# aconverse/ffmpeg-heaac

Measured on AMD Instinct MI355X. Metric: HE-AAC frames/s (batched), higher is better.
Workload: dtype f32; 1 GPU; HE-AACv2 stereo 48 kHz, 256 k-frame batch; frames_per_gpu=262144, pcm=f32, bytes_per_frame=85284, parallelism=frames sharded by index, no collective

## Files before the change

### ffmpeg-heaac_amd/csrc/k_he.hip

```cpp
#include <stdlib.h>
#include <type_traits>
#include "k_core.h"
#include "k_core2.h"
#include "kernels.h"

#include "k_hf.h"

#define ANA_WAVES 8
#define ANA_POOL  3456

struct AnaLds {
    CoreLds core;
    float qmf_ds[320];
    float rot[64];
    float pool[ANA_WAVES][ANA_POOL];
};

__device__ __forceinline__ void qmf_analysis_wave(const float *qmf_ds, const float *rot,
                                                  const float *c16, const float *c32,
                                                  const float *x, float *u, float *g_W, int lane)
{
    {
        const int k = lane;
        const float w0 = qmf_ds[k], w1 = qmf_ds[k + 64], w2 = qmf_ds[k + 128],
                    w3 = qmf_ds[k + 192], w4 = qmf_ds[k + 256];
        for (int i = 0; i < 32; i++) {
            const float *xs = x + 32 * i + 319 - k;
            const float f = w0 * xs[0] + w1 * xs[-64] + w2 * xs[-128] + w3 * xs[-192] + w4 * xs[-256];
            u[i * 65 + k] = f;
        }
    }
    wave_sync();
    if (lane < 32) {
        const float *f = u + lane * 65;
        float o[64];
        imdct128_reg([&](int j) -> float {
                         if (j == 0)  return f[0];
                         if (j == 63) return f[32];
                         return (j & 1) ? f[(j + 1) >> 1] : -f[64 - (j >> 1)];
                     }, o, rot, c16, c32);
        float *row = u + lane * 65;
#pragma unroll
        for (int k = 0; k < 32; k++) {
            row[2 * k]     = -o[63 - k];
            row[2 * k + 1] = o[k];
        }
    }
    wave_sync();
    for (int t = lane; t < 2048; t += WAVE)
        g_W[t] = u[(t >> 6) * 65 + (t & 63)];
    wave_sync();
}

#define CA_WAVES 7
#define CA_U     2080

struct CaWave {
    float tu[2 * 2 * C2_TSTRIDE];
    float x1[1312];
    float x0u1[CA_U];
};
static_assert(CA_U >= 1312, "x of channel 0 fits under u of channel 1");
static_assert(CA_U <= 2 * 2 * C2_TSTRIDE, "u rows of channel 0 lie over the core's transpose regions");

template <bool STRIDED, class... Hold>
__global__ __launch_bounds__(CA_WAVES * WAVE)
void k_core_ana(const float *__restrict__ g_tab, const uint16_t *__restrict__ g_rev,
                const float *__restrict__ g_coeffs, const HeaacIcs *__restrict__ g_ics,
                const float *g_state_in, float *g_state_out, int state_words,
                int ncore, int off_saved0, int off_sbr0,
                float *__restrict__ g_W, float scale, unsigned long long n_units, unsigned long long rstride, Hold... hold)
{
    constexpr bool HOLD = sizeof...(Hold) != 0;
    static_assert(STRIDED || !HOLD, "the batch form has no hold mask");
    auto rec = [&](unsigned long long u) -> unsigned long long {
        if constexpr (STRIDED) return (u / ncore) * rstride * ncore + u % ncore;
        else return u;
    };
    __shared__ float s_cos[TB_ROT2048];
    __shared__ float s_rot256[128];
    __shared__ float s_wshort[256];
    __shared__ uint16_t s_kA512[512], s_kA64[64];
    __shared__ float s_qmf_ds[320];
    __shared__ float s_rot[64];
    __shared__ CaWave S[CA_WAVES];
    static_assert(TB_SINE_SHORT == TB_KBD_SHORT + 128, "the two short windows are copied as one run");
    for (int i = threadIdx.x; i < TB_ROT2048; i += blockDim.x) s_cos[i] = g_tab[i];
    for (int i = threadIdx.x; i < 128; i += blockDim.x) s_rot256[i] = g_tab[TB_ROT256 + i];
    for (int i = threadIdx.x; i < 256; i += blockDim.x) s_wshort[i] = g_tab[TB_KBD_SHORT + i];
    for (int k = threadIdx.x; k < 512; k += blockDim.x) {
        const int e = g_rev[RV_512 + k];
        s_kA512[(e & 15) * 32 + (e >> 4)] = (uint16_t)k;
    }
    for (int k = threadIdx.x; k < 64; k += blockDim.x) {
        const int e = g_rev[RV_64 + k];
        s_kA64[(e & 15) * 4 + (e >> 4)] = (uint16_t)k;
    }
    for (int i = threadIdx.x; i < 320; i += blockDim.x) s_qmf_ds[i] = g_tab[TB_QMF_DS + i];
    for (int i = threadIdx.x; i < 64; i += blockDim.x)  s_rot[i] = g_tab[TB_ROT128A + i];
    __syncthreads();
    const CoreTabs L = { s_cos, g_tab + TB_ROT2048, s_rot256, g_tab + TB_KBD_LONG, g_tab + TB_SINE_LONG,
                         s_wshort, s_wshort + 128,
                         reinterpret_cast<const float2 *>(g_tab + TB_ROTA512), reinterpret_cast<const float2 *>(g_tab + TB_ROTA64),
                         s_kA512, s_kA64 };
    const int wave = __builtin_amdgcn_readfirstlane(threadIdx.x / WAVE), lane0 = threadIdx.x % WAVE;
    CaWave &w = S[wave];
    cpx *T0 = reinterpret_cast<cpx *>(w.tu), *T1 = T0 + C2_TSTRIDE;
    const float *c16 = s_cos + TB_COS16, *c32 = s_cos + TB_COS32;
    const unsigned long long pairs = (n_units + 1) / 2;
    LongTw tw;
    core2_load_long_twiddles(L, lane0 & 31, tw);
    for (unsigned long long pr = (unsigned long long)blockIdx.x * CA_WAVES + wave; pr < pairs;
         pr += (unsigned long long)gridDim.x * CA_WAVES) {
        const unsigned long long u0 = 2 * pr;
        const bool have1 = u0 + 1 < n_units;
        const unsigned long long u1 = have1 ? u0 + 1 : u0;
        unsigned long long r0 = rec(u0), r1 = rec(u1);
        [[maybe_unused]] bool run0 = true, run1 = have1;
        if constexpr (HOLD) {
            const uint8_t *g_hold = hold_mask(hold...);
            run0 = __builtin_amdgcn_readfirstlane((int)g_hold[(u0 / ncore) * rstride]) == 0;
            run1 = have1 && __builtin_amdgcn_readfirstlane((int)g_hold[(u1 / ncore) * rstride]) == 0;
            if (!run0 && !run1) continue;
            if (!run0) r0 = r1;
            if (!run1) r1 = r0;
        }
        const HeaacIcs ics0 = g_ics[r0], ics1 = g_ics[r1];
        int lane = opaque(lane0);
        core2_stage_coeffs(reinterpret_cast<float *>(T0), g_coeffs + r0 * 1024, lane);
        core2_stage_coeffs(reinterpret_cast<float *>(T1), g_coeffs + r1 * 1024, lane);
        wave_sync();
        {
            const int half = lane >> 5, hl = lane & 31;
            const bool eight = (half ? ics1.window_sequence[0] : ics0.window_sequence[0]) == HEAAC_EIGHT_SHORT_SEQUENCE;
            cpx *T = half ? T1 : T0;
            imdct_half_regs_tw<true>(L, reinterpret_cast<const float *>(T), T, eight, hl, tw);
        }
#pragma unroll
        for (int c = 0; c < 2; c++) {
            if (c == 1 && !have1) break;
            if constexpr (HOLD) {
                if (!(c ? run1 : run0)) continue;
            }
            const unsigned long long u = c ? u1 : u0;
            const unsigned long long f = u / ncore;
            const int ch = (int)(u - f * ncore);
            const float *st_in = g_state_in + f * state_words;
            float *st_out = g_state_out + f * state_words;
            const int off_saved = off_saved0 + ch * HEAAC_ST_SAVED;
            const int off_sbr = off_sbr0 + ch * HEAAC_ST_SBR;
            float *x = c ? w.x1 : w.x0u1;
            const float *xh_in = st_in + off_sbr + HEAAC_SBR_XHIST;
            float xh[5];
#pragma unroll
            for (int t = 0; t < 5; t++) xh[t] = 64 * t + lane < 288 ? xh_in[64 * t + lane] : 0.0f;
            const float *buf = reinterpret_cast<const float *>(c ? T1 : T0);
            const OverlapHbm ov{ st_in + off_saved, st_out + off_saved };
            if (scale != 1.0f)
                core2_window(L, c ? ics1 : ics0, 0.0f, buf, ov, lane, [&](int q, float v) { x[288 + q] = v * scale; });
            else
                core2_window(L, c ? ics1 : ics0, 0.0f, buf, ov, lane, [&](int q, float v) { x[288 + q] = v; });
#pragma unroll
            for (int t = 0; t < 5; t++) if (64 * t + lane < 288) x[64 * t + lane] = xh[t];
        }
        wave_sync();
        lane = opaque(lane);
#pragma unroll
        for (int c = 0; c < 2; c++) {
            if (c == 1 && !have1) break;
            if constexpr (HOLD) {
                if (!(c ? run1 : run0)) continue;
            }
            const unsigned long long u = c ? u1 : u0;
            const unsigned long long f = u / ncore;
            const int ch = (int)(u - f * ncore);
            float *xh_out = g_state_out + f * state_words + off_sbr0 + ch * HEAAC_ST_SBR + HEAAC_SBR_XHIST;
            const float *x = c ? w.x1 : w.x0u1;
            float *uu = c ? w.x0u1 : w.tu;
#pragma unroll
            for (int t = 0; t < 5; t++) if (64 * t + lane < 288) xh_out[64 * t + lane] = x[1024 + 64 * t + lane];
            const int k = lane;
            const float w0 = s_qmf_ds[k], w1 = s_qmf_ds[k + 64], w2 = s_qmf_ds[k + 128],
                        w3 = s_qmf_ds[k + 192], w4 = s_qmf_ds[k + 256];
            const float *xk = x + 319 - k;
            v2f a1 = v2f{xk[-64], xk[-32]}, a2 = v2f{xk[-128], xk[-96]}, a3 = v2f{xk[-192], xk[-160]},
                a4 = v2f{xk[-256], xk[-224]};
#pragma unroll
            for (int i = 0; i < 32; i += 2) {
                const v2f a0 = v2f{xk[32 * i], xk[32 * i + 32]};
                const v2f f = bc(w0) * a0 + bc(w1) * a1 + bc(w2) * a2 + bc(w3) * a3 + bc(w4) * a4;
                uu[i * 65 + k] = f.x;
                uu[(i + 1) * 65 + k] = f.y;
                a4 = a3; a3 = a2; a2 = a1; a1 = a0;
            }
        }
        wave_sync();
        lane = opaque(lane);
        {
            float *row = (lane >> 5 ? w.x0u1 : w.tu) + (lane & 31) * 65;
            const float *f = row;
            float o[64];
            imdct128_reg([&](int j) -> float {
                             if (j == 0)  return f[0];
                             if (j == 63) return f[32];
                             return (j & 1) ? f[(j + 1) >> 1] : -f[64 - (j >> 1)];
                         }, o, s_rot, c16, c32);
#pragma unroll
            for (int k = 0; k < 32; k++) {
                row[2 * k]     = -o[63 - k];
                row[2 * k + 1] = o[k];
            }
        }
        wave_sync();
#pragma unroll
        for (int c = 0; c < 2; c++) {
            if (c == 1 && !have1) break;
            if constexpr (HOLD) {
                if (!(c ? run1 : run0)) continue;
            }
            const float *uu = c ? w.x0u1 : w.tu;
            float *Wo = g_W + (c ? u1 : u0) * 2048;
#pragma unroll
            for (int it = 0; it < 8; it++) {
                const int r = 4 * it + (lane >> 4), q = 4 * (lane & 15);
                const float *sr = uu + r * 65 + q;
                *reinterpret_cast<float4 *>(Wo + r * 64 + q) = make_float4(sr[0], sr[1], sr[2], sr[3]);
            }
        }
        wave_sync();
    }
}

template <bool STRIDED, class... Hold>
__global__ __launch_bounds__(HF_WAVES * WAVE)
void k_hfadj(const float *__restrict__ g_tab,
             const HeaacSbrFrame *__restrict__ g_sbr, const HeaacSbrHeader *__restrict__ g_hdr, unsigned n_hdr,
             const float *g_W, const float *g_state_in, float *g_state_out, int state_words,
             int ncore, int off_sbr0, float *g_X, unsigned long long n_units, unsigned *g_queue,
             unsigned char *__restrict__ g_xtop, unsigned long long rstride, Hold... hold)
{
    static_assert(STRIDED || sizeof...(Hold) == 0, "the batch form has no hold mask");
    __shared__ float s_xlow[HF_WAVES][HF_XLOW_WORDS], s_aux[HF_WAVES][HF_AUX_WORDS], s_rec[HF_WAVES][HF_REC_WORDS];
    __shared__ float s_noise[1024];
    wg_copy_f4(s_noise, g_tab + TB_NOISE, 1024);
    __syncthreads();
    const int wave = __builtin_amdgcn_readfirstlane(threadIdx.x / WAVE), lane = threadIdx.x % WAVE;
    const HfWave S = hf_wave_view(s_xlow[wave], s_aux[wave], s_rec[wave]);
    FrameFeed<1> feed;
    feed.init((unsigned long long)blockIdx.x * HF_WAVES + wave, (unsigned long long)gridDim.x * HF_WAVES, g_queue, lane);
    while (feed.cur * 2 < n_units) {
        const unsigned long long ub = feed.cur * 2;
        feed.request(lane);
      for (int qi = 0; qi < 2 && ub + qi < n_units; qi++) {
        const unsigned long long u = ub + qi;
        const unsigned long long f = u / ncore;
        if constexpr (sizeof...(Hold) != 0) {
            if (__builtin_amdgcn_readfirstlane((int)hold_mask(hold...)[f * rstride])) continue;
        }
        const int ch = (int)(u - f * ncore);
        const int off = off_sbr0 + ch * HEAAC_ST_SBR;
        const HeaacSbrFrame *sbr = STRIDED ? &g_sbr[f * rstride] : &g_sbr[f];
        v2f *Xc = reinterpret_cast<v2f *>(g_X + (f * 2 + ch) * HE_X_CHANNEL);
        int xb = 64;
        hf_channel(S, s_noise, sbr, g_hdr, n_hdr, ch, g_W + u * 2048,
                   g_state_in + f * state_words + off, g_state_out + f * state_words + off, lane,
                   [&](int i, float re, float im) {
                       if (i == 0 && g_xtop) {
                           const int top16 = (S.h.kx + S.h.m + 15) & ~15;
                           const int t_old = S.c[ch].t_env_num_env_old;
                           const bool zero = 2 * t_old - 32 <= 0 || (int)sbr->kx_old + (int)sbr->m_old <= top16;
                           xb = __builtin_amdgcn_readfirstlane(zero && top16 < 64 ? top16 : 64);
                           if (lane == 0 && xb != 64) g_xtop[f * 2 + ch] = (unsigned char)xb;
                       }
                       if (lane < xb) __builtin_nontemporal_store(v2f{re, im}, Xc + i * 64 + lane);
                   });
      }
        feed.advance();
    }
}

#define SYN_WAVES 6
#define VB_STRIDE 129
#define VB_ROWS   41

#define SYN_WAVES_F32 7
struct SynWave {
    __attribute__((aligned(16))) float vb[VB_ROWS * VB_STRIDE + 3];
};
template <int NW>
struct SynLdsT {
    float win[640];
    float rot[64];
    float c16[8], c32[12];
    SynWave w[NW];
};
typedef SynLdsT<SYN_WAVES> SynLds;

#ifdef HEAAC_STAMPS
#define SSTAMP(i) TL_STAMP(i, (i) == 0)
#else
#define SSTAMP(i) do {} while (0)
#endif

__device__ __forceinline__ float lane_xor1(float v)
{
    return __int_as_float(__builtin_amdgcn_update_dpp(0, __float_as_int(v), 0xB1, 0xF, 0xF, false));
}

struct SynIn {
// ... 499 lines not shown
#pragma nounroll
                        for (int q = lane; q < 1024; q += WAVE) o[q * nout] = 0;
                    }
                    continue;
                }
                move = fresh;
                fresh = true;
            }
            if (move) {
                float h[9];
#pragma unroll
                for (int k = 0; k < 9; k++) h[k] = vb[k * DS_STRIDE + lane];
#pragma unroll
                for (int k = 0; k < 9; k++) vb[(32 + k) * DS_STRIDE + lane] = h[k];
            }
            const unsigned long long u = (unsigned long long)t * n_streams + st, r = st * T + t;
            const float *X0 = g_X + (u * 2 + ch) * HE_X_CHANNEL;
            if constexpr (FMT == HEAAC_PCM_F32_PLANAR) {
                float *o = reinterpret_cast<float *>(g_pcm) + (r * nout + ch) * 1024;
                synth_ds_channel<false, false>(S, vb, X0, nullptr, nullptr, nullptr, scale, bias, lane,
                                               [&](int i, int nn, float v) { o[32 * i + nn] = v; });
            } else {
                int16_t *o = reinterpret_cast<int16_t *>(g_pcm) + r * 1024 * nout + ch;
                synth_ds_channel<false, false>(S, vb, X0, nullptr, nullptr, nullptr, scale, bias, lane,
                                               [&](int i, int nn, float v) { o[(32 * i + nn) * nout] = (int16_t)pcm_int16<FMT>(v); });
            }
        }
        if constexpr (HOLD) {
            const int row0 = fresh ? 0 : 32;
            for (int q = lane; q < 576; q += WAVE) v_out[q] = vb[(row0 + (q >> 6)) * DS_STRIDE + (q & 63)];
        } else {
            for (int q = lane; q < 576; q += WAVE) v_out[q] = vb[(q >> 6) * DS_STRIDE + (q & 63)];
        }
        wave_sync();
    }
}

static int he_grid(unsigned long long units, int per_block)
{
    unsigned long long g = (units + per_block - 1) / per_block;
    if (g > 256) g = 256;
    if (g < 1) g = 1;
    return (int)g;
}

static bool he_fused()
{
#ifdef HEAAC_TUNING
    static const bool fused = []() { const char *e = getenv("HEAAC_HE_UNFUSED"); return !(e && e[0] == '1'); }();
    return fused;
#else
    return true;
#endif
}

extern "C" int heaac_launch_he(const float *d_tab, const uint16_t *d_rev, int cfg,
                               const float *d_coeffs, const HeaacIcs *d_ics,
                               const HeaacSbrFrame *d_sbr, const HeaacSbrHeader *d_hdr, unsigned n_hdr,
                               const HeaacPsFrame *d_ps,
                               const float *d_state_in, float *d_state_out,
                               void *d_pcm, int pcm_format,
                               float *d_ws_W, float *d_ws_X, unsigned *d_queue,
                               unsigned char *d_xtop, const float *d_zero,
                               size_t n, size_t pcm_frame0, int flags, hipStream_t s)
{
    const int ncore = cfg == HEAAC_CFG_HEV1 ? 2 : 1;
    const int nout  = cfg == HEAAC_CFG_HEV1_MONO ? 1 : 2;
    int words, off_saved0 = 0, off_sbr0, off_syn0;
    if (cfg == HEAAC_CFG_HEV1) {
        words = HEAAC_STATE_WORDS_HEV1; off_sbr0 = 2 * HEAAC_ST_SAVED; off_syn0 = off_sbr0 + 2 * HEAAC_ST_SBR;
    } else if (cfg == HEAAC_CFG_HEV1_MONO) {
        words = HEAAC_STATE_WORDS_HEV1_MONO; off_sbr0 = HEAAC_ST_SAVED; off_syn0 = off_sbr0 + HEAAC_ST_SBR;
    } else if (cfg == HEAAC_CFG_HEV2) {
        words = HEAAC_STATE_WORDS_HEV2; off_sbr0 = HEAAC_ST_SAVED; off_syn0 = off_sbr0 + HEAAC_ST_SBR;
    } else
        return HEAAC_ERR_ARG;
    const unsigned long long units = (unsigned long long)n * ncore;
    const bool simd = pcm_format == HEAAC_PCM_S16_INTERLEAVED_SSE2;
    const float sf_scale = simd ? -1.0f / 1024.0f : HEAAC_SF_SCALE;

    if (hipMemsetAsync(d_queue, 0, 64, s) != hipSuccess) return HEAAC_ERR_HIP;
    if (hipMemsetAsync(d_xtop, 64, 2 * n, s) != hipSuccess) return HEAAC_ERR_HIP;
    hipLaunchKernelGGL(k_core_ana<false>, dim3(he_grid((units + 1) / 2, CA_WAVES)), dim3(CA_WAVES * WAVE), 0, s,
                       d_tab, d_rev, d_coeffs, d_ics, d_state_in, d_state_out, words, ncore,
                       off_saved0, off_sbr0, d_ws_W, 1 / (-1024 * sf_scale), units, 1ull);
    if (cfg == HEAAC_CFG_HEV2 && he_fused()) {
        const int off_ps = off_syn0 + 2 * HEAAC_ST_SYNTH;
        int rc = heaac_launch_hfps(d_tab, d_sbr, d_hdr, n_hdr, d_ps, d_ws_W, d_state_in, d_state_out, words,
                                   off_sbr0, off_ps, d_ws_X, n, d_queue, d_xtop, 1, nullptr, s);
        if (rc != HEAAC_OK) return rc;
        rc = heaac_launch_ps(d_tab, d_ps, d_sbr, d_hdr, n_hdr, d_state_in, d_state_out, words, off_ps, d_ws_X, n, 2, 1, nullptr, s);
        if (rc != HEAAC_OK) return rc;
    } else {
        hipLaunchKernelGGL(k_hfadj<false>, dim3(he_grid((units + 1) / 2, HF_WAVES)), dim3(HF_WAVES * WAVE), 0, s,
                           d_tab, d_sbr, d_hdr, n_hdr, d_ws_W, d_state_in, d_state_out, words, ncore, off_sbr0,
                           d_ws_X, units, d_queue + 1, cfg == HEAAC_CFG_HEV2 ? nullptr : d_xtop, 1ull);
        if (cfg == HEAAC_CFG_HEV2) {
            int rc = heaac_launch_ps(d_tab, d_ps, d_sbr, d_hdr, n_hdr, d_state_in, d_state_out, words,
                                     off_syn0 + 2 * HEAAC_ST_SYNTH, d_ws_X, n, 3, 1, nullptr, s);
            if (rc != HEAAC_OK) return rc;
        }
    }
    const float scale = -1024 * sf_scale, bias = simd ? 0.0f : HEAAC_ADD_BIAS;
    if (flags & HEAAC_HE_DOWNSAMPLED) {
        const dim3 gd(he_grid(n, DS_WAVES)), bd(DS_WAVES * WAVE);
        char *pcm = (char *)d_pcm + pcm_frame0 * nout * 1024 * (pcm_format == HEAAC_PCM_F32_PLANAR ? 4 : 2);
        if (pcm_format == HEAAC_PCM_F32_PLANAR)
            hipLaunchKernelGGL((k_synth_ds<HEAAC_PCM_F32_PLANAR>), gd, bd, 0, s, d_tab, d_ws_X, d_state_in, d_state_out,
                               words, off_syn0, nout, (void *)pcm, scale, bias, (unsigned long long)n);
        else if (simd)
            hipLaunchKernelGGL((k_synth_ds<HEAAC_PCM_S16_INTERLEAVED_SSE2>), gd, bd, 0, s, d_tab, d_ws_X, d_state_in, d_state_out,
                               words, off_syn0, nout, (void *)pcm, scale, bias, (unsigned long long)n);
        else
            hipLaunchKernelGGL((k_synth_ds<HEAAC_PCM_S16_INTERLEAVED>), gd, bd, 0, s, d_tab, d_ws_X, d_state_in, d_state_out,
                               words, off_syn0, nout, (void *)pcm, scale, bias, (unsigned long long)n);
        return hipGetLastError() == hipSuccess ? HEAAC_OK : HEAAC_ERR_HIP;
    }
    const dim3 g(he_grid(n, SYN_WAVES_F32)), b(SYN_WAVES_F32 * WAVE);
    if (pcm_format == HEAAC_PCM_F32_PLANAR)
        hipLaunchKernelGGL((k_synth<HEAAC_PCM_F32_PLANAR>), g, b, 0, s, d_tab, d_ws_X, d_state_in, d_state_out,
                           words, off_syn0, nout, d_pcm, scale, bias,
                           (unsigned long long)n, (unsigned long long)pcm_frame0, d_queue + 2, d_xtop, d_zero);
    else if (pcm_format == HEAAC_PCM_S16_INTERLEAVED)
        hipLaunchKernelGGL((k_synth<HEAAC_PCM_S16_INTERLEAVED>), g, b, 0, s, d_tab, d_ws_X, d_state_in, d_state_out,
                           words, off_syn0, nout, d_pcm, scale, bias,
                           (unsigned long long)n, (unsigned long long)pcm_frame0, d_queue + 2, d_xtop, d_zero);
    else if (simd)
        hipLaunchKernelGGL((k_synth<HEAAC_PCM_S16_INTERLEAVED_SSE2>), g, b, 0, s, d_tab, d_ws_X, d_state_in, d_state_out,
                           words, off_syn0, nout, d_pcm, scale, bias,
                           (unsigned long long)n, (unsigned long long)pcm_frame0, d_queue + 2, d_xtop, d_zero);
    else
        return HEAAC_ERR_ARG;
    return hipGetLastError() == hipSuccess ? HEAAC_OK : HEAAC_ERR_HIP;
}

#define HE_LAUNCH_STREAMS(PLAIN, HOLD, mask, grid, block, ...)                                        \
    do {                                                                                          \
        const uint8_t *he_mask_ = (mask);                                                         \
        if (he_mask_) hipLaunchKernelGGL(HOLD, grid, block, 0, s, __VA_ARGS__, he_mask_);         \
        else hipLaunchKernelGGL(PLAIN, grid, block, 0, s, __VA_ARGS__);                           \
    } while (0)

extern "C" int heaac_launch_he_streams(const float *d_tab, const uint16_t *d_rev, int cfg,
                                       const float *d_coeffs, const HeaacIcs *d_ics,
                                       const HeaacSbrFrame *d_sbr, const HeaacSbrHeader *d_hdr, unsigned n_hdr,
                                       const HeaacPsFrame *d_ps,
                                       const float *d_state_in, float *d_state_out,
                                       void *d_pcm, int pcm_format,
                                       float *d_ws_W, float *d_ws_X, unsigned *d_queue,
                                       unsigned char *d_xtop, const float *d_zero,
                                       size_t n_streams, size_t T, int flags, const uint8_t *d_hold, hipStream_t s)
{
    const int ncore = cfg == HEAAC_CFG_HEV1 ? 2 : 1;
    const int nout  = cfg == HEAAC_CFG_HEV1_MONO ? 1 : 2;
    int words, off_saved0 = 0, off_sbr0, off_syn0;
    if (cfg == HEAAC_CFG_HEV1) {
        words = HEAAC_STATE_WORDS_HEV1; off_sbr0 = 2 * HEAAC_ST_SAVED; off_syn0 = off_sbr0 + 2 * HEAAC_ST_SBR;
    } else if (cfg == HEAAC_CFG_HEV1_MONO) {
        words = HEAAC_STATE_WORDS_HEV1_MONO; off_sbr0 = HEAAC_ST_SAVED; off_syn0 = off_sbr0 + HEAAC_ST_SBR;
    } else if (cfg == HEAAC_CFG_HEV2) {
        words = HEAAC_STATE_WORDS_HEV2; off_sbr0 = HEAAC_ST_SAVED; off_syn0 = off_sbr0 + HEAAC_ST_SBR;
    } else
        return HEAAC_ERR_ARG;
    if (!n_streams || !T) return HEAAC_OK;
    const unsigned long long units = (unsigned long long)n_streams * ncore;
    const bool simd = pcm_format == HEAAC_PCM_S16_INTERLEAVED_SSE2;
    const float sf_scale = simd ? -1.0f / 1024.0f : HEAAC_SF_SCALE;
    if (hipMemsetAsync(d_xtop, 64, 2 * n_streams * T, s) != hipSuccess) return HEAAC_ERR_HIP;
    if (d_hold && d_state_in != d_state_out) {
        if (hipMemcpyAsync(d_state_out, d_state_in, n_streams * (size_t)words * sizeof(float), hipMemcpyDeviceToDevice, s) != hipSuccess)
            return HEAAC_ERR_HIP;
        d_state_in = d_state_out;
    }
    for (size_t t = 0; t < T; t++) {
        const float *st_in = t ? d_state_out : d_state_in;
        float *W = d_ws_W + t * units * 2048;
        float *X = d_ws_X + t * n_streams * 2 * HE_X_CHANNEL;
        unsigned char *xtop = d_xtop + 2 * t * n_streams;
        HE_LAUNCH_STREAMS((k_core_ana<true>), (k_core_ana<true, const uint8_t *>), d_hold ? d_hold + t : nullptr,
                          dim3(he_grid((units + 1) / 2, CA_WAVES)), dim3(CA_WAVES * WAVE),
                          d_tab, d_rev, d_coeffs + t * ncore * 1024, d_ics + t * ncore, st_in, d_state_out, words, ncore,
                          off_saved0, off_sbr0, W, 1 / (-1024 * sf_scale), units, (unsigned long long)T);
        if (hipMemsetAsync(d_queue, 0, 64, s) != hipSuccess) return HEAAC_ERR_HIP;
        if (cfg == HEAAC_CFG_HEV2) {
            const int off_ps = off_syn0 + 2 * HEAAC_ST_SYNTH;
            int rc = heaac_launch_hfps(d_tab, d_sbr + t, d_hdr, n_hdr, d_ps + t, W, st_in, d_state_out, words,
                                       off_sbr0, off_ps, X, n_streams, d_queue, xtop, T, d_hold ? d_hold + t : nullptr, s);
            if (rc != HEAAC_OK) return rc;
            rc = heaac_launch_ps(d_tab, d_ps + t, d_sbr + t, d_hdr, n_hdr, st_in, d_state_out, words, off_ps, X,
                                 n_streams, 2, T, d_hold ? d_hold + t : nullptr, s);
            if (rc != HEAAC_OK) return rc;
        } else {
            HE_LAUNCH_STREAMS((k_hfadj<true>), (k_hfadj<true, const uint8_t *>), d_hold ? d_hold + t : nullptr,
                              dim3(he_grid((units + 1) / 2, HF_WAVES)), dim3(HF_WAVES * WAVE),
                              d_tab, d_sbr + t, d_hdr, n_hdr, W, st_in, d_state_out, words, ncore, off_sbr0,
                              X, units, d_queue + 1, xtop, (unsigned long long)T);
        }
    }
    const float scale = -1024 * sf_scale, bias = simd ? 0.0f : HEAAC_ADD_BIAS;
    const unsigned long long chains = (unsigned long long)n_streams * nout;
    const unsigned long long ns = n_streams;
    const unsigned Tu = (unsigned)T;
    if (flags & HEAAC_HE_DOWNSAMPLED) {
        const dim3 gd(he_grid(chains, DS_WAVES)), bd(DS_WAVES * WAVE);
#define SYN_DS(FMT) \
        HE_LAUNCH_STREAMS((k_synth_ds_streams<FMT>), (k_synth_ds_streams<FMT, const uint8_t *>), d_hold, gd, bd, d_tab, d_ws_X, \
                          d_state_in, d_state_out, words, off_syn0, nout, d_pcm, scale, bias, ns, Tu)
        if (pcm_format == HEAAC_PCM_F32_PLANAR) SYN_DS(HEAAC_PCM_F32_PLANAR);
        else if (simd) SYN_DS(HEAAC_PCM_S16_INTERLEAVED_SSE2);
        else SYN_DS(HEAAC_PCM_S16_INTERLEAVED);
#undef SYN_DS
        return hipGetLastError() == hipSuccess ? HEAAC_OK : HEAAC_ERR_HIP;
    }
    const dim3 g(he_grid(chains, SYN_WAVES_F32)), b(SYN_WAVES_F32 * WAVE);
#define SYN(FMT) \
    HE_LAUNCH_STREAMS((k_synth_streams<FMT>), (k_synth_streams<FMT, const uint8_t *>), d_hold, g, b, d_tab, d_ws_X, d_state_in, \
                      d_state_out, words, off_syn0, nout, d_pcm, scale, bias, ns, Tu, d_queue + 2, d_xtop, d_zero)
    if (pcm_format == HEAAC_PCM_F32_PLANAR) SYN(HEAAC_PCM_F32_PLANAR);
    else if (pcm_format == HEAAC_PCM_S16_INTERLEAVED) SYN(HEAAC_PCM_S16_INTERLEAVED);
    else if (simd) SYN(HEAAC_PCM_S16_INTERLEAVED_SSE2);
    else return HEAAC_ERR_ARG;
#undef SYN
    return hipGetLastError() == hipSuccess ? HEAAC_OK : HEAAC_ERR_HIP;
}

extern "C" int heaac_launch_qmf_analysis(const float *d_tab, const float *d_in, const float *d_xh_in,
                                         float *d_xh_out, float *d_W, float scale, size_t n, hipStream_t s)
{
    if (!n) return HEAAC_OK;
    hipLaunchKernelGGL(k_qmf_analysis, dim3(he_grid(n, ANA_WAVES)), dim3(ANA_WAVES * WAVE), 0, s,
                       d_tab, d_in, d_xh_in, d_xh_out, d_W, scale, (unsigned long long)n);
    return hipGetLastError() == hipSuccess ? HEAAC_OK : HEAAC_ERR_HIP;
}

extern "C" int heaac_launch_qmf_synthesis(const float *d_tab, const float *d_X, const float *d_v_in,
                                          float *d_v_out, float *d_out, float scale, float bias,
                                          size_t n, hipStream_t s)
{
    if (!n) return HEAAC_OK;
    hipLaunchKernelGGL(k_qmf_synthesis, dim3(he_grid(n, SYN_WAVES)), dim3(SYN_WAVES * WAVE), 0, s,
                       d_tab, d_X, d_v_in, d_v_out, d_out, scale, bias, (unsigned long long)n);
    return hipGetLastError() == hipSuccess ? HEAAC_OK : HEAAC_ERR_HIP;
}

extern "C" int heaac_launch_qmf_synthesis_ds(const float *d_tab, const float *d_X, const float *d_v_in,
                                            float *d_v_out, float *d_out, float scale, float bias,
                                            size_t n, hipStream_t s)
{
    if (n == 0) return HEAAC_OK;
    hipLaunchKernelGGL(k_qmf_synthesis_ds, dim3(he_grid(n, DS_WAVES)), dim3(DS_WAVES * WAVE), 0, s,
                       d_tab, d_X, d_v_in, d_v_out, d_out, scale, bias, (unsigned long long)n);
    return hipGetLastError() == hipSuccess ? HEAAC_OK : HEAAC_ERR_HIP;
}


#ifdef HEAAC_STAMPS
extern "C" int heaac_debug_timeline_he(unsigned long long *out)
{
    if (hipMemcpyFromSymbol(out, HIP_SYMBOL(g_tl_acc), sizeof(g_tl_acc)) != hipSuccess) return -1;
    return hipMemcpyFromSymbol(out + 32, HIP_SYMBOL(g_tl_cnt), sizeof(g_tl_cnt)) == hipSuccess ? 0 : -1;
}
#endif
```

### ffmpeg-heaac_amd/csrc/k_hf.h

```cpp
#pragma once
#include "k_common.h"
#include "heaac_dsp.h"

#define ENV_ADJ 2

#ifdef HEAAC_STAMPS
static __device__ unsigned long long g_tl_acc[32], g_tl_last[256], g_tl_cnt;
#define TL_STAMP(i, is_first) do { wave_sync(); \
    if (lane == 0 && (blockIdx.x & 7) == 7 && threadIdx.x < 64) { \
        const unsigned long long t_ = __builtin_readcyclecounter(), l_ = g_tl_last[blockIdx.x]; \
        if (is_first) { if (l_) atomicAdd(&g_tl_acc[31], t_ - l_); atomicAdd(&g_tl_cnt, 1ull); } \
        else atomicAdd(&g_tl_acc[i], t_ - l_); \
        g_tl_last[blockIdx.x] = t_; } } while (0)
#define HSTAMP(i) TL_STAMP(i, (i) == 0)
#else
#define HSTAMP(i) do {} while (0)
#endif

__device__ __forceinline__ float exp2_half_normal(int twice)
{
    const int e = twice >> 1;
    const unsigned mant = (twice & 1) ? 0x3FB504F3u : 0x3F800000u;
    return __uint_as_float(mant + ((unsigned)e << 23));
}
// ... 29 lines not shown
                   reinterpret_cast<float (*)[2]>(aux + 8 + MAXE * MAXM), reinterpret_cast<float (*)[2]>(aux + 8 + MAXE * MAXM + 64),
                   aux,
                   reinterpret_cast<float (*)[MAXM]>(aux + 8),
                   reinterpret_cast<float (*)[MAXM]>(aux + 8 + MAXE * MAXM),
                   reinterpret_cast<float (*)[32]>(aux + 8 + 2 * MAXE * MAXM),
                   *reinterpret_cast<HeaacSbrHeader *>(rec),
                   reinterpret_cast<HeaacSbrChannel *>(rec + sizeof(HeaacSbrHeader) / 4) };
}

__device__ __forceinline__ void lds_copy_bytes(void *dst, const void *src, int bytes, int lane)
{
    const uint32_t *s = reinterpret_cast<const uint32_t *>(src);
    uint32_t *d = reinterpret_cast<uint32_t *>(dst);
    for (int i = lane; i < bytes / 4; i += WAVE) d[i] = s[i];
}

__device__ __forceinline__ float deq_env(const HfWave &w, int coupling, int ch, int e, int i)
{
    if (coupling) {
        const int amp = w.c[0].bs_amp_res;
        const int q0 = w.c[0].env_facs_q[e][i], q1 = w.c[1].env_facs_q[e][i];
        const float temp1 = exp2_half(amp ? 2 * q0 + 14 : q0 + 14);
        const float temp2 = exp2_half(amp ? 2 * (12 - q1) : 24 - q1);
        const float fac = temp1 / (1.0f + temp2);
        return ch ? fac * temp2 : fac;
    }
    const int amp = w.c[ch].bs_amp_res;
    const int q = w.c[ch].env_facs_q[e][i];
    return exp2_half((amp ? 2 * q : q) + 12);
}

__device__ __forceinline__ float deq_noise(const HfWave &w, int coupling, int ch, int e, int i)
{
    if (coupling) {
        const int q0 = w.c[0].noise_facs_q[e][i], q1 = w.c[1].noise_facs_q[e][i];
        const float temp1 = exp2_half(2 * (7 - q0));
        const float temp2 = exp2_half(2 * (12 - q1));
        const float fac = temp1 / (1.0f + temp2);
        return ch ? fac * temp2 : fac;
    }
    return exp2_half(2 * (6 - (int)w.c[ch].noise_facs_q[e][i]));
}

#define FFMIN_(a, b) ((a) > (b) ? (b) : (a))

__device__ __forceinline__ void xhigh3(float2 x2, float2 x1, float2 x0, const float *a, float &re, float &im)
{
    re = x2.x * a[0] - x2.y * a[1] + x1.x * a[2] - x1.y * a[3] + x0.x;
    im = x2.y * a[0] + x2.x * a[1] + x1.y * a[2] + x1.x * a[3] + x0.y;
}
__device__ __forceinline__ v2f swp(v2f a) { return __builtin_shufflevector(a, a, 1, 0); }
__device__ __forceinline__ v2f xhigh3_pk(v2f x2, v2f x1, v2f x0, const float *a)
{
    v2f t = bc(a[0]) * x2;
    t = t + v2f{-a[1], a[1]} * swp(x2);
    t = t + bc(a[2]) * x1;
    t = t + v2f{-a[3], a[3]} * swp(x1);
    return t + x0;
}

template <class Emit, class Hook = NoHook>
__device__ __forceinline__ void hf_channel(const HfWave &w, const float *g_noise ,
                                           const HeaacSbrFrame *g_fr, const HeaacSbrHeader *g_hdr, unsigned n_hdr,
                                           int ch, const float *g_W,
                                           const float *st_in, float *st_out, int lane_in, Emit emit,
                                           Hook after_params = Hook())
{
    const int lane = opaque(lane_in);
    HSTAMP(0);
    const int hdr_idx = g_fr->hdr < n_hdr ? g_fr->hdr : n_hdr - 1;
    uint32_t creg[3], hreg[3];
    {
        const uint32_t *cs = reinterpret_cast<const uint32_t *>(&g_fr->ch[0]);
        const uint32_t *hs_ = reinterpret_cast<const uint32_t *>(&g_hdr[hdr_idx]);
#pragma unroll
        for (int r = 0; r < 3; r++) {
            creg[r] = lane + 64 * r < 168 ? cs[lane + 64 * r] : 0;
            hreg[r] = lane + 64 * r < 133 ? hs_[lane + 64 * r] : 0;
        }
    }
    const int start = g_fr->start, reset = g_fr->reset;
    const int kx_old = g_fr->kx_old, m_old = g_fr->m_old;
    const int coupling = g_fr->bs_coupling;
    float2 wreg[16], treg[4];
    {
        const float2 *W2 = reinterpret_cast<const float2 *>(g_W);
        const float2 *T2 = reinterpret_cast<const float2 *>(st_in + HEAAC_SBR_WTAIL);
#pragma unroll
        for (int r = 0; r < 16; r++) wreg[r] = W2[lane + 64 * r];
#pragma unroll
        for (int r = 0; r < 4; r++) treg[r] = T2[lane + 64 * r];
    }
    const int k = lane;
    float ghist[4], qhist[4];
    unsigned idxnoise = __float_as_uint(st_in[HEAAC_SBR_IDXNOISE]);
    unsigned idxsine  = __float_as_uint(st_in[HEAAC_SBR_IDXSINE]);
    const float bw_in = lane < 5 ? st_in[HEAAC_SBR_BW + lane] : 0.0f;
    {
        uint32_t *cd = reinterpret_cast<uint32_t *>(&w.c[0]);
        uint32_t *hd = reinterpret_cast<uint32_t *>(&w.h);
#pragma unroll
        for (int r = 0; r < 3; r++) {
            if (lane + 64 * r < 168) cd[lane + 64 * r] = creg[r];
            if (lane + 64 * r < 133) hd[lane + 64 * r] = hreg[r];
        }
    }
    after_params();
    wave_sync();
    const HeaacSbrHeader &h = w.h;
    const HeaacSbrChannel &c = w.c[ch];
    const int kx = h.kx, m_max = h.m, n_q = h.n_q;
    const int m = k - kx;
    const bool in_sbr = m >= 0 && m < m_max && m < MAXM;
    const int num_env = c.bs_num_env;
    const int t0 = c.t_env[0], tL = c.t_env[num_env];
    const int h_SL = 4 * !h.bs_smoothing_mode;
#pragma unroll
    for (int j = 0; j < 4; j++) {
        ghist[j] = in_sbr ? st_in[HEAAC_SBR_GTAIL + j * MAXM + m] : 0.0f;
        qhist[j] = in_sbr ? st_in[HEAAC_SBR_QTAIL + j * MAXM + m] : 0.0f;
    }
    const int sidx0 = in_sbr ? reinterpret_cast<const uint8_t *>(st_in + HEAAC_SBR_SIDX)[m] : 0;
    if (reset) idxnoise = 0;

    HSTAMP(1);
    {
#pragma unroll
        for (int r = 0; r < 16; r++) {
            const int t = lane + 64 * r, i = t >> 5, kk = t & 31;
            float2 v = wreg[r];
            if (kk >= kx) v = make_float2(0.0f, 0.0f);
            float *d = w.xlow + kk * XL_STRIDE + 2 * (i + 8);
            d[0] = v.x; d[1] = v.y;
        }
#pragma unroll
        for (int r = 0; r < 4; r++) {
            const int t = lane + 64 * r, i = t >> 5, kk = t & 31;
            float2 v = treg[r];
            if (kk >= kx_old) v = make_float2(0.0f, 0.0f);
            float *d = w.xlow + kk * XL_STRIDE + 2 * i;
            d[0] = v.x; d[1] = v.y;
        }
        float2 *To = reinterpret_cast<float2 *>(st_out + HEAAC_SBR_WTAIL);
#pragma unroll
        for (int r = 0; r < 4; r++) To[lane + 64 * r] = wreg[12 + r];
    }
    if (lane < 8) w.bw[lane] = bw_in;
    wave_sync();

    float e_orig[MAXE], q_map[MAXE], e_curr[MAXE], gain[MAXE], q_m[MAXE], s_m[MAXE];
    int sidx[MAXE];
    unsigned smap = 0;
    float kc[4] = { 0, 0, 0, 0 };
#pragma unroll
    for (int e = 0; e < MAXE; e++) { e_orig[e] = q_map[e] = e_curr[e] = gain[e] = q_m[e] = s_m[e] = 0.0f; sidx[e] = 0; }
    const int p_src = in_sbr ? (int)h.map_src[k] : 0xff;
    const bool has_src = p_src < 32;
    const int row = k < kx ? (k < 32 ? k : 0) : (has_src ? p_src : 0);
    const float2 *xr = reinterpret_cast<const float2 *>(0);
    (void)xr;
    const float *xrow = w.xlow + row * XL_STRIDE;

    if (start) {
        HSTAMP(2);
        {
            const int band_in_pass = (lane * 171) >> 9;
            const int lag = lane - 3 * band_in_pass;
            const int k0 = h.k0 < 32 ? h.k0 : 32;
            for (int first = 0; first < k0; first += 21) {
                const int band = first + band_in_pass;
                const bool active = lane < 63 && band < k0;
                const float *xs = w.xlow + (active ? band : 0) * XL_STRIDE;
                const float *xl = xs + 2 * lag;
                float s0 = 0.0f, s1 = 0.0f;
#pragma unroll
                for (int i = 1; i < 38; i++) {
                    const float a = xs[2 * i], b = xs[2 * i + 1], c = xl[2 * i], d = xl[2 * i + 1];
                    s0 += a * c + b * d;
                    s1 += a * d - b * c;
                }
                const float lo0 = s0 + xs[0] * xl[0] + xs[1] * xl[1];
                const float lo1 = s1 + xs[0] * xl[1] - xs[1] * xl[0];
                const float hi0 = s0 + xs[76] * xl[76] + xs[77] * xl[77];
                const float hi1 = s1 + xs[76] * xl[77] - xs[77] * xl[76];
                const int l1 = lane + 1 < 64 ? lane + 1 : 63, l2 = lane + 2 < 64 ? lane + 2 : 63;
                const float p110 = __shfl(lo0, l1), p111 = __shfl(lo1, l1), p000 = __shfl(hi0, l1), p001 = __shfl(hi1, l1);
                const float p010 = __shfl(lo0, l2), p011 = __shfl(lo1, l2);
                if (active && lag == 0) {
                    const float p210 = lo0, p100 = hi0;
                    const float dk = p210 * p100 - (p110 * p110 + p111 * p111) / 1.000001f;
                    float a1r, a1i, a0r, a0i;
                    if (!dk) {
                        a1r = 0; a1i = 0;
                    } else {
                        const float tr = p000 * p110 - p001 * p111 - p010 * p100;
                        const float ti = p000 * p111 + p001 * p110 - p011 * p100;
                        a1r = tr / dk;
                        a1i = ti / dk;
                    }
                    if (!p100) {
                        a0r = 0; a0i = 0;
                    } else {
                        const float tr = p000 + a1r * p110 + a1i * p111;
                        const float ti = p001 + a1i * p110 - a1r * p111;
                        a0r = -tr / p100;
                        a0i = -ti / p100;
                    }
                    if (a1r * a1r + a1i * a1i >= 16.0f || a0r * a0r + a0i * a0i >= 16.0f) {
                        a1r = 0; a1i = 0; a0r = 0; a0i = 0;
                    }
                    w.alpha0[band][0] = a0r; w.alpha0[band][1] = a0i;
                    w.alpha1[band][0] = a1r; w.alpha1[band][1] = a1i;
                }
            }
        }
        HSTAMP(3);
        if (lane < n_q) {
            const int m0 = c.bs_invf_mode[0][lane], m1 = c.bs_invf_mode[1][lane];
            float new_bw;
            if (m0 + m1 == 1) new_bw = 0.6f;
            else new_bw = m0 == 0 ? 0.0f : m0 == 1 ? 0.75f : m0 == 2 ? 0.9f : 0.98f;
            const float old = w.bw[lane];
            if (new_bw < old) new_bw = 0.75f    * new_bw + 0.25f    * old;
            else              new_bw = 0.90625f * new_bw + 0.09375f * old;
            w.bw[lane] = new_bw < 0.015625f ? 0.0f : new_bw;
        }
        wave_sync();

// ... 381 lines not shown
```

### ffmpeg-heaac_amd/csrc/k_hfr.h

```cpp
#pragma once
#include "k_hf.h"

#define HFR_REC_WORDS ((int)((sizeof(HeaacSbrHeader) + sizeof(HeaacSbrChannel)) / 4))

__device__ __forceinline__ float lane_get(int addr, float v)
{
    return __int_as_float(__builtin_amdgcn_ds_bpermute(addr, __float_as_int(v)));
}
__device__ __forceinline__ v2f lane_get2(int addr, v2f v)
{
    return v2f{lane_get(addr, v.x), lane_get(addr, v.y)};
}

__device__ __forceinline__ bool hf_frame_is_fast(const HeaacSbrFrame *g_fr, const HeaacSbrHeader *g_hdr, unsigned n_hdr)
{
    const unsigned hi = g_fr->hdr;
    const HeaacSbrHeader &h = g_hdr[hi < n_hdr ? hi : n_hdr - 1];
    return g_fr->start && h.bs_interpol_freq && !g_fr->bs_coupling;
}

template <class Hook = NoHook>
__device__ __forceinline__ void hf_channel_rx(const HfWave &w, const float *g_noise ,
                                              const HeaacSbrFrame *g_fr, const HeaacSbrHeader *g_hdr, unsigned n_hdr,
                                              const float *g_W, const float *st_in, float *st_out, int lane_in,
                                              v2f (&xl)[40], Hook after_params = Hook())
{
    const int lane = opaque(lane_in);
    HSTAMP(0);
    const int hdr_idx = g_fr->hdr < n_hdr ? g_fr->hdr : n_hdr - 1;
    uint32_t creg[2], hreg[3];
    {
        const uint32_t *cs = reinterpret_cast<const uint32_t *>(&g_fr->ch[0]);
        const uint32_t *hs_ = reinterpret_cast<const uint32_t *>(&g_hdr[hdr_idx]);
#pragma unroll
        for (int r = 0; r < 2; r++) creg[r] = lane + 64 * r < 84 ? cs[lane + 64 * r] : 0;
#pragma unroll
        for (int r = 0; r < 3; r++) hreg[r] = lane + 64 * r < 133 ? hs_[lane + 64 * r] : 0;
    }
    const int reset = g_fr->reset;
    const int kx_old = g_fr->kx_old, m_old = g_fr->m_old;
    const int k = lane;
    {
        const GBuf Wb(g_W), Tb(st_in);
        const int kb = opaque((lane & 31) * 8);
        const v2f zero = {0.0f, 0.0f};
#pragma unroll
        for (int i = 0; i < 40; i++) xl[i] = zero;
        if (lane < 32) {
#pragma unroll
            for (int i = 24; i < 32; i++) xl[8 + i] = Wb.ldb2(kb, i * 64);
#pragma unroll
            for (int i = 0; i < 24; i++) xl[8 + i] = Wb.ldb2(kb, i * 64);
#pragma unroll
            for (int i = 0; i < 8; i++) xl[i] = Tb.ldb2(kb, HEAAC_SBR_WTAIL + i * 64);
        }
    }
    unsigned idxnoise = __float_as_uint(st_in[HEAAC_SBR_IDXNOISE]);
    unsigned idxsine  = __float_as_uint(st_in[HEAAC_SBR_IDXSINE]);
    const float bw_in = lane < 5 ? st_in[HEAAC_SBR_BW + lane] : 0.0f;
    {
        uint32_t *cd = reinterpret_cast<uint32_t *>(&w.c[0]);
        uint32_t *hd = reinterpret_cast<uint32_t *>(&w.h);
#pragma unroll
        for (int r = 0; r < 2; r++) if (lane + 64 * r < 84) cd[lane + 64 * r] = creg[r];
#pragma unroll
        for (int r = 0; r < 3; r++) if (lane + 64 * r < 133) hd[lane + 64 * r] = hreg[r];
    }
    after_params();
    wave_sync();
    const HeaacSbrHeader &h = w.h;
    const HeaacSbrChannel &c = w.c[0];
    const int kx = h.kx, m_max = h.m, n_q = h.n_q;
    const int m = k - kx;
    const bool in_sbr = m >= 0 && m < m_max && m < MAXM;
    const int num_env = c.bs_num_env;
    const int t0 = c.t_env[0], tL = c.t_env[num_env];
    const int h_SL = 4 * !h.bs_smoothing_mode;
    const int sidx0 = in_sbr ? reinterpret_cast<const uint8_t *>(st_in + HEAAC_SBR_SIDX)[m] : 0;
    if (reset) idxnoise = 0;

    HSTAMP(1);
    {
        const GBufT<0> To(st_out);
        if (lane < 32) {
#pragma unroll
            for (int j = 0; j < 8; j++) To.stb2(xl[32 + j], opaque(lane * 8), HEAAC_SBR_WTAIL + j * 64);
        }
        const v2f zero = {0.0f, 0.0f};
#pragma unroll
        for (int i = 0; i < 32; i++) xl[8 + i] = k >= kx ? zero : xl[8 + i];
#pragma unroll
        for (int i = 0; i < 8; i++) xl[i] = k >= kx_old ? zero : xl[i];
    }
    if (lane < 8) w.bw[lane] = bw_in;
    wave_sync();

    float e_orig[MAXE], q_map[MAXE], e_curr[MAXE], gain[MAXE], q_m[MAXE], s_m[MAXE];
    int sidx[MAXE];
    unsigned smap = 0;
    float kc[4] = { 0, 0, 0, 0 };
#pragma unroll
    for (int e = 0; e < MAXE; e++) { e_orig[e] = q_map[e] = e_curr[e] = gain[e] = q_m[e] = s_m[e] = 0.0f; sidx[e] = 0; }
    const int p_src = in_sbr ? (int)h.map_src[k] : 0xff;
    const bool has_src = p_src < 32;
    const int src_addr = (has_src ? p_src : lane) * 4;
    const int t_old = c.t_env_num_env_old;
    const int i_Temp = 2 * t_old - 32 > 0 ? 2 * t_old - 32 : 0;

    {
        HSTAMP(2);
        float a0r = 0.0f, a0i = 0.0f, a1r = 0.0f, a1i = 0.0f;
        {
            float r0 = 0.0f;
            v2f s1 = {0.0f, 0.0f}, s2 = {0.0f, 0.0f};
#pragma unroll
            for (int i = 1; i < 38; i++) {
                const v2f x = xl[i];
                r0 += x.x * x.x + x.y * x.y;
                { const v2f y = xl[i + 1]; s1.x += x.x * y.x + x.y * y.y; s1.y += x.x * y.y - x.y * y.x; }
                { const v2f y = xl[i + 2]; s2.x += x.x * y.x + x.y * y.y; s2.y += x.x * y.y - x.y * y.x; }
                __builtin_amdgcn_sched_barrier(0);
            }
            auto edge = [](v2f s, v2f x, v2f y) {
                return v2f{s.x + x.x * y.x + x.y * y.y, s.y + x.x * y.y - x.y * y.x};
            };
            const float p210 = r0 + xl[0].x * xl[0].x + xl[0].y * xl[0].y;
            const float p100 = r0 + xl[38].x * xl[38].x + xl[38].y * xl[38].y;
            const v2f lo1 = edge(s1, xl[0], xl[1]), hi1 = edge(s1, xl[38], xl[39]);
            const v2f lo2 = edge(s2, xl[0], xl[2]);
            const float p110 = lo1.x, p111 = lo1.y, p000 = hi1.x, p001 = hi1.y, p010 = lo2.x, p011 = lo2.y;
            const float dk = p210 * p100 - (p110 * p110 + p111 * p111) / 1.000001f;
            if (dk != 0.0f) {
                const float tr = p000 * p110 - p001 * p111 - p010 * p100;
                const float ti = p000 * p111 + p001 * p110 - p011 * p100;
                a1r = tr / dk;
// ... 347 lines not shown
```

Before: 26.21 million frames/s.

## Split QMF analysis output into low/high halves and skip high-band writes when kx<=16

The analysis kernel now writes the 32-subband QMF matrix W as two 16-subband halves in a split layout. It looks ahead to each pair's SBR header to get kx, and when kx<=16 it skips storing most of the upper half. The HF consumers (k_hf.h and k_hfr.h) are updated to read the new layout and to skip loading the upper-subband rows when kx<=16, which cuts global memory traffic. The cost is an extra prefetch of the header per pair and more indexing complexity. There is also a risk of layout mismatch with any other reader of W.

Result: faster. 26.53 million frames/s, median of 6 (+1.2%).

```diff
diff --git a/ffmpeg-heaac_amd/csrc/k_he.hip b/ffmpeg-heaac_amd/csrc/k_he.hip
--- a/ffmpeg-heaac_amd/csrc/k_he.hip
+++ b/ffmpeg-heaac_amd/csrc/k_he.hip
@@ -67,6 +67,7 @@
 __global__ __launch_bounds__(CA_WAVES * WAVE)
 void k_core_ana(const float *__restrict__ g_tab, const uint16_t *__restrict__ g_rev,
                 const float *__restrict__ g_coeffs, const HeaacIcs *__restrict__ g_ics,
+                const HeaacSbrFrame *__restrict__ g_sbr, const HeaacSbrHeader *__restrict__ g_hdr, unsigned n_hdr,
                 const float *g_state_in, float *g_state_out, int state_words,
                 int ncore, int off_saved0, int off_sbr0,
                 float *__restrict__ g_W, float scale, unsigned long long n_units, unsigned long long rstride, Hold... hold)
@@ -110,8 +111,20 @@
     const unsigned long long pairs = (n_units + 1) / 2;
     LongTw tw;
     core2_load_long_twiddles(L, lane0 & 31, tw);
-    for (unsigned long long pr = (unsigned long long)blockIdx.x * CA_WAVES + wave; pr < pairs;
-         pr += (unsigned long long)gridDim.x * CA_WAVES) {
+    auto pair_hdr = [&](unsigned long long p) -> unsigned {
+        unsigned long long u = 2 * p + (opaque(lane0) & 1);
+        if (u >= n_units) u = n_units - 1;
+        const unsigned long long f = ncore == 2 ? u >> 1 : ncore == 1 ? u : u / ncore;
+        const unsigned hi = g_sbr[STRIDED ? f * rstride : f].hdr;
+        return hi < n_hdr ? hi : n_hdr - 1;
+    };
+    auto hdr_kx = [&](unsigned hi) -> unsigned { return g_hdr[hi].kx; };
+    const unsigned long long pr_first = (unsigned long long)blockIdx.x * CA_WAVES + wave;
+    const unsigned long long pr_step = (unsigned long long)gridDim.x * CA_WAVES;
+    unsigned kxv = pr_first < pairs ? hdr_kx(pair_hdr(pr_first)) : 0;
+    for (unsigned long long pr = pr_first; pr < pairs; pr += pr_step) {
+        const unsigned hdr_next = pair_hdr(pr + pr_step);
+        const unsigned kx_now = kxv;
         const unsigned long long u0 = 2 * pr;
         const bool have1 = u0 + 1 < n_units;
         const unsigned long long u1 = have1 ? u0 + 1 : u0;
@@ -121,7 +134,7 @@
             const uint8_t *g_hold = hold_mask(hold...);
             run0 = __builtin_amdgcn_readfirstlane((int)g_hold[(u0 / ncore) * rstride]) == 0;
             run1 = have1 && __builtin_amdgcn_readfirstlane((int)g_hold[(u1 / ncore) * rstride]) == 0;
-            if (!run0 && !run1) continue;
+            if (!run0 && !run1) { kxv = hdr_kx(hdr_next); continue; }
             if (!run0) r0 = r1;
             if (!run1) r1 = r0;
         }
@@ -165,6 +178,7 @@
         }
         wave_sync();
         lane = opaque(lane);
+        kxv = hdr_kx(hdr_next);
 #pragma unroll
         for (int c = 0; c < 2; c++) {
             if (c == 1 && !have1) break;
@@ -212,6 +226,7 @@
             }
         }
         wave_sync();
+        const bool cut0 = __builtin_amdgcn_readlane((int)kx_now, 0) <= 16, cut1 = __builtin_amdgcn_readlane((int)kx_now, 1) <= 16;
 #pragma unroll
         for (int c = 0; c < 2; c++) {
             if (c == 1 && !have1) break;
@@ -220,11 +235,16 @@
             }
             const float *uu = c ? w.x0u1 : w.tu;
             float *Wo = g_W + (c ? u1 : u0) * 2048;
-#pragma unroll
-            for (int it = 0; it < 8; it++) {
-                const int r = 4 * it + (lane >> 4), q = 4 * (lane & 15);
-                const float *sr = uu + r * 65 + q;
-                *reinterpret_cast<float4 *>(Wo + r * 64 + q) = make_float4(sr[0], sr[1], sr[2], sr[3]);
+            const bool cut = c ? cut1 : cut0;
+#pragma unroll
+            for (int p = 0; p < 2; p++) {
+#pragma unroll
+                for (int it = 0; it < 4; it++) {
+                    if (p == 1 && it < 3 && cut) continue;
+                    const int r = 8 * it + (lane >> 3), q = 4 * (lane & 7);
+                    const float *sr = uu + r * 65 + 32 * p + q;
+                    *reinterpret_cast<float4 *>(Wo + 1024 * p + r * 32 + q) = make_float4(sr[0], sr[1], sr[2], sr[3]);
+                }
             }
         }
         wave_sync();
@@ -890,7 +910,7 @@
     if (hipMemsetAsync(d_queue, 0, 64, s) != hipSuccess) return HEAAC_ERR_HIP;
     if (hipMemsetAsync(d_xtop, 64, 2 * n, s) != hipSuccess) return HEAAC_ERR_HIP;
     hipLaunchKernelGGL(k_core_ana<false>, dim3(he_grid((units + 1) / 2, CA_WAVES)), dim3(CA_WAVES * WAVE), 0, s,
-                       d_tab, d_rev, d_coeffs, d_ics, d_state_in, d_state_out, words, ncore,
+                       d_tab, d_rev, d_coeffs, d_ics, d_sbr, d_hdr, n_hdr, d_state_in, d_state_out, words, ncore,
                        off_saved0, off_sbr0, d_ws_W, 1 / (-1024 * sf_scale), units, 1ull);
     if (cfg == HEAAC_CFG_HEV2 && he_fused()) {
         const int off_ps = off_syn0 + 2 * HEAAC_ST_SYNTH;
@@ -987,7 +1007,8 @@
         unsigned char *xtop = d_xtop + 2 * t * n_streams;
         HE_LAUNCH_STREAMS((k_core_ana<true>), (k_core_ana<true, const uint8_t *>), d_hold ? d_hold + t : nullptr,
                           dim3(he_grid((units + 1) / 2, CA_WAVES)), dim3(CA_WAVES * WAVE),
-                          d_tab, d_rev, d_coeffs + t * ncore * 1024, d_ics + t * ncore, st_in, d_state_out, words, ncore,
+                          d_tab, d_rev, d_coeffs + t * ncore * 1024, d_ics + t * ncore, d_sbr + t, d_hdr, n_hdr, st_in,
+                          d_state_out, words, ncore,
                           off_saved0, off_sbr0, W, 1 / (-1024 * sf_scale), units, (unsigned long long)T);
         if (hipMemsetAsync(d_queue, 0, 64, s) != hipSuccess) return HEAAC_ERR_HIP;
         if (cfg == HEAAC_CFG_HEV2) {
diff --git a/ffmpeg-heaac_amd/csrc/k_hf.h b/ffmpeg-heaac_amd/csrc/k_hf.h
--- a/ffmpeg-heaac_amd/csrc/k_hf.h
+++ b/ffmpeg-heaac_amd/csrc/k_hf.h
@@ -135,14 +135,23 @@
     const int start = g_fr->start, reset = g_fr->reset;
     const int kx_old = g_fr->kx_old, m_old = g_fr->m_old;
     const int coupling = g_fr->bs_coupling;
+    const bool w_cut = __builtin_amdgcn_readfirstlane((int)g_hdr[hdr_idx].kx) <= 16;
     float2 wreg[16], treg[4];
     {
         const float2 *W2 = reinterpret_cast<const float2 *>(g_W);
         const float2 *T2 = reinterpret_cast<const float2 *>(st_in + HEAAC_SBR_WTAIL);
 #pragma unroll
-        for (int r = 0; r < 16; r++) wreg[r] = W2[lane + 64 * r];
+        for (int r = 0; r < 8; r++) wreg[r] = W2[lane + 64 * r];
+#pragma unroll
+        for (int r = 14; r < 16; r++) wreg[r] = W2[lane + 64 * r];
 #pragma unroll
         for (int r = 0; r < 4; r++) treg[r] = T2[lane + 64 * r];
+#pragma unroll
+        for (int r = 8; r < 14; r++) wreg[r] = make_float2(0.0f, 0.0f);
+        if (!w_cut) {
+#pragma unroll
+            for (int r = 8; r < 14; r++) wreg[r] = W2[lane + 64 * r];
+        }
     }
     const int k = lane;
     float ghist[4], qhist[4];
@@ -180,7 +189,7 @@
     {
 #pragma unroll
         for (int r = 0; r < 16; r++) {
-            const int t = lane + 64 * r, i = t >> 5, kk = t & 31;
+            const int i = 4 * (r & 7) + (lane >> 4), kk = 16 * (r >> 3) + (lane & 15);
             float2 v = wreg[r];
             if (kk >= kx) v = make_float2(0.0f, 0.0f);
             float *d = w.xlow + kk * XL_STRIDE + 2 * (i + 8);
@@ -196,7 +205,10 @@
         }
         float2 *To = reinterpret_cast<float2 *>(st_out + HEAAC_SBR_WTAIL);
 #pragma unroll
-        for (int r = 0; r < 4; r++) To[lane + 64 * r] = wreg[12 + r];
+        for (int r = 0; r < 4; r++) {
+            const int i = 4 * (r & 1) + (lane >> 4), kk = 16 * (r >> 1) + (lane & 15);
+            To[i * 32 + kk] = wreg[6 + (r & 1) + 8 * (r >> 1)];
+        }
     }
     if (lane < 8) w.bw[lane] = bw_in;
     wave_sync();
diff --git a/ffmpeg-heaac_amd/csrc/k_hfr.h b/ffmpeg-heaac_amd/csrc/k_hfr.h
--- a/ffmpeg-heaac_amd/csrc/k_hfr.h
+++ b/ffmpeg-heaac_amd/csrc/k_hfr.h
@@ -42,15 +42,18 @@
     const int k = lane;
     {
         const GBuf Wb(g_W), Tb(st_in);
-        const int kb = opaque((lane & 31) * 8);
+        const int kb = opaque((lane & 31) * 8), kw = opaque(((lane >> 4) & 1) * 4096 + (lane & 15) * 8);
+        const bool w_cut = g_hdr[hdr_idx].kx <= 16;
         const v2f zero = {0.0f, 0.0f};
 #pragma unroll
         for (int i = 0; i < 40; i++) xl[i] = zero;
         if (lane < 32) {
 #pragma unroll
-            for (int i = 24; i < 32; i++) xl[8 + i] = Wb.ldb2(kb, i * 64);
-#pragma unroll
-            for (int i = 0; i < 24; i++) xl[8 + i] = Wb.ldb2(kb, i * 64);
+            for (int i = 24; i < 32; i++) xl[8 + i] = Wb.ldb2(kw, i * 32);
+            if (lane < 16 || !w_cut) {
+#pragma unroll
+                for (int i = 0; i < 24; i++) xl[8 + i] = Wb.ldb2(kw, i * 32);
+            }
 #pragma unroll
             for (int i = 0; i < 8; i++) xl[i] = Tb.ldb2(kb, HEAAC_SBR_WTAIL + i * 64);
         }
```
